# NeuralRevenant/RASSEngine

Measured on AMD Instinct MI355X. Metric: queries/sec, exact cosine top-10 over N x 1024-d fp32 corpus in HBM, higher is better.
Workload: dtype f32; 1 GPU; 1000000 x 1024-d flat cosine top-10, 1 x MI355X, precomputed embeddings (BASELINE configs[1]); rows_per_gpu=1000000, rows_global=1000000, dim=1024, k=10, query_batch=32, corpus_dtype=f32, layout=tile16, mode=flat

## Files before the change

rassengine_amd/csrc/api_internal.h:

```cpp
#pragma once

#include <hip/hip_runtime.h>
#include <stdint.h>
#include <stdio.h>
#include <stdlib.h>
#include <string.h>
#include <unistd.h>

#include <algorithm>
#include <atomic>
#include <condition_variable>
#include <map>
#include <mutex>
#include <new>
#include <string>
#include <type_traits>
#include <vector>

#include "../../include/rass_engine.h"
#include "kernels.h"

namespace rass {
namespace host {

// ... 334 lines not shown
    int64_t* d_pair_ids = nullptr;
    unsigned char* d_batch = nullptr;
    size_t batch_bytes = 0;
    unsigned char* d_allow_ws = nullptr;
    size_t allow_ws_bytes = 0;
};

namespace rass {
namespace host {

int set_device(const rass_engine* eng);
int index_reserve(rass_index* idx, int64_t need_rows);
void index_free_slabs(rass_index* idx);
int index_attr_ensure(rass_index* idx, int col);
int index_refresh_copies(rass_index* idx, int64_t first, int64_t n, hipStream_t st);

int scan_xcd_skew(int nq, int grid, int n_cus);
int64_t scan_sample_floor_min_share();
bool i8_sample_floor(int64_t rows, int grid);
enum { kBatchSampleGroups = 0, kBatchSampleF32 = 1, kBatchSampleRep = 2 };
int scan_batch_sample_mode();
bool scan_batch_pair();
bool scan_batch_step();
bool ivf_batch_one_launch();

int scan_grid(int64_t tiles, int lists_kept_per_wg, int n_cus);

template <class F>
int timed_launch(rass_engine* eng, hipStream_t st, F&& launch, int extra_groups = 0) {
    const bool timed = eng && eng->ev_on && (size_t)(2 * eng->ev_used + 1) < eng->ev_pool.size();
    if (timed) HIP_TRY(hipEventRecord(eng->ev_pool[2 * eng->ev_used], st));
    const int rc = launch();
    if (rc != RASS_OK) return rc;
    if (timed) {
        HIP_TRY(hipEventRecord(eng->ev_pool[2 * eng->ev_used + 1], st));
        eng->ev_used += 1;
        eng->ev_extra += extra_groups;
    }
    return RASS_OK;
}

inline void as_sample(rass::ScanArgs& s) { s.xcd_skew = 0, s.sample_pass = true; }
inline void as_sample(rass::ScanBf16Args& s) { s.k = 1; }
inline void as_sample(rass::ScanI8Args& s) { s.k = 1; }
template <class Args>
int sample_prelaunch(Args& a, int grid, float* best, hipError_t (*launch)(const Args&, int, hipStream_t), hipStream_t st,
// ... 174 lines not shown
```

rassengine_amd/csrc/api_scan.hip:

```cpp

#include "api_internal.h"

namespace rass {
namespace host {


int scan_xcd_skew(int nq, int grid, int n_cus) {
    struct Skew {
        int b16 = 4, b32 = 0;
        Skew() {
            if (const char* e = getenv("RASS_SCAN_XCD_SKEW")) {
                int a = 0, b = 0;
                const int n = sscanf(e, "%d,%d", &a, &b);
                if (n == 1) b = a;
                if (n >= 1 && a >= 0 && b >= 0 && a <= 4096 && b <= 4096) b16 = a, b32 = b;
            }
        }
    };
    if (grid != n_cus || grid % 8 != 0) return 0;
    static const Skew skew;
    return nq <= 16 ? skew.b16 : skew.b32;
}

int64_t scan_sample_floor_min_share() {
// ... 9 lines not shown
    if (e && !force && atoi(e) == 0) return false;
    return grid <= rass::kMaxSampleGroups && rows >= (int64_t)(force ? 2 : 8) * 64 * grid;
}

int scan_batch_sample_mode() {
    const char* e = getenv("RASS_SCAN_BATCH_SAMPLE");
    if (e && e[0] == 'g') return kBatchSampleGroups;
    if (e && e[0] == 'f') return kBatchSampleF32;
    return kBatchSampleRep;
}

bool scan_batch_pair() {
    static const bool on = [] {
        const char* e = getenv("RASS_SCAN_BATCH_PAIR");
        return !(e && e[0] == '0');
    }();
    return on;
}

bool scan_batch_step() {
    const char* e = getenv("RASS_SCAN_BATCH_STEP");
    return !(e && e[0] == '0');
}

bool ivf_batch_one_launch() {
    const char* e = getenv("RASS_IVF_BATCH_FINE");
    return !(e && e[0] == 'g');
}


int scan_grid(int64_t tiles, int lists_kept_per_wg, int n_cus) {
    int grid = (int)std::min<int64_t>(std::max<int64_t>(tiles, 1), std::min(n_cus, kMaxGrid));
    if ((int64_t)grid * lists_kept_per_wg > rass::kMergeMaxCandidates) grid = rass::kMergeMaxCandidates / lists_kept_per_wg;
    return grid;
}

ScratchView scratch_layout(unsigned char* base, int nq, int k) {
    Carver c{base};
    ScratchView L;
    L.q_padded = c.take<float>((size_t)RASS_MAX_QBATCH * kMaxStride * sizeof(float));
    L.part_scores = c.take<float>((size_t)kMaxGrid * nq * k * sizeof(float));
    L.part_ids = c.take<int64_t>((size_t)kMaxGrid * nq * k * sizeof(int64_t));
    L.q_bf16 = c.take<unsigned short>((size_t)RASS_MAX_QBATCH * kMaxStride * 2);
    L.cand_scores = c.take<float>((size_t)RASS_MAX_QBATCH * RASS_MAX_K * sizeof(float));
    L.cand_ids = c.take<int64_t>((size_t)RASS_MAX_QBATCH * RASS_MAX_K * sizeof(int64_t));
    L.sample_best = c.take<float>((size_t)rass::kMaxSampleGroups * 32 * sizeof(float));
// ... 436 lines not shown
```

rassengine_amd/csrc/api_search.hip:

```cpp

#include "api_internal.h"

namespace rass {
namespace host {

HostSlot* slot_acquire(rass_engine* eng) {
    std::unique_lock<std::mutex> lk(eng->slot_mu);
    for (;;) {
        for (HostSlot& sl : eng->slots)
            if (!sl.busy) {
                sl.busy = true;
                return &sl;
            }
        eng->slot_cv.wait(lk);
    }
}

void slot_release(rass_engine* eng, HostSlot* sl) {
    {
        std::lock_guard<std::mutex> lk(eng->slot_mu);
        sl->busy = false;
    }
    eng->slot_cv.notify_one();
}
// ... 81 lines not shown
    hipStream_t st = eng->stream;
    const int nq = r.nq, k = r.k;
    const IndexView iv = index_view(idx, r.q_filter != nullptr, r.id_base);
    const int64_t rows = iv.rows;
    const int64_t stride = idx->stride;
    if (int rc = check_k(k)) return rc;
    if (rows < 0 || rows > kMaxScanRows) return fail(RASS_ERR_INVALID, "n_rows out of range for one scan");
    if (!rass::scan_supported_stride(stride) || stride > kMaxStride)
        return fail(RASS_ERR_UNSUPPORTED, kStrideMsg);
    const int groups = (nq + RASS_MAX_QBATCH - 1) / RASS_MAX_QBATCH;
    if (stride > kNarrowStride) {
        for (int g = 0; g < groups; ++g) {
            const int rc = search_device_group(idx, batch_group(idx, r, g, gs, gi));
            if (rc != RASS_OK) return rc;
        }
        return RASS_OK;
    }
    const BatchSamplePlan plan = batch_sample_plan(eng, rows, stride, nq, k);
    const int grid = plan.grid;
    int rc = grow_block(&eng->d_batch, &eng->batch_bytes, batch_layout(nullptr, groups, grid, k, stride).total, st);
    if (rc != RASS_OK) return rc;
    const BatchView L = batch_layout(eng->d_batch, groups, grid, k, stride);

    HIP_TRY(rass::launch_normalize_rows_f32(r.queries, idx->dim, L.q_padded, stride, nq, idx->dim, st, (int64_t)groups * 32));

    auto group_args = [&](int g) {
        rass::ScanArgs a;
        a.corpus = iv.corpus;
        a.row_tag = iv.row_tag;
        a.q_padded = L.q_padded + (int64_t)g * 32 * stride;
        a.q_filter = r.q_filter ? r.q_filter + g * 32 : nullptr;
        a.part_scores = L.part_scores + (int64_t)g * L.part_per_group;
        a.part_ids = L.part_ids + (int64_t)g * L.part_per_group;
        a.row_stride = stride;
        a.id_base = iv.id_base;
        a.n_rows = (int)rows;
        a.nq = std::min(RASS_MAX_QBATCH, nq - g * 32);
        a.k = k;
        a.xcd_skew = scan_xcd_skew(a.nq, grid, eng->n_cus);
        return a;
    };
    const int64_t sample_rows = (int64_t)64 * grid;
    const bool sample = plan.sample, one_sample = plan.one_sample;
    const int sample_wgs = one_sample ? 32 : grid;
    if (plan.rep) {
        HIP_TRY(rass::launch_sample_rep(iv.corpus, iv.row_tag, stride, grid, L.q_padded, r.q_filter, nq, L.rep_qfrag, L.rep_part,
                                        L.rep_row, L.sample_best, st));
    } else if (one_sample) {
        rass::ScanArgs s = group_args(0);
        s.n_rows = (int)sample_rows;
        s.xcd_skew = 0;
        s.sample_pass = true;
        s.nq = 32;
        s.part_scores = L.sample_best;
        s.part_ids = nullptr;
        s.wgs_per_group = sample_wgs;
        s.q_group_stride = 32 * stride;
        s.part_group_stride = (int64_t)32 * rass::kMaxSampleGroups;
        s.nq_total = nq;
        HIP_TRY(rass::launch_scan_topk_f32(s, groups * sample_wgs, st));
    } else if (sample)
        for (int g = 0; g < groups; ++g) {
            rass::ScanArgs a = group_args(g);
            if (a.nq <= 16) continue;
            rc = sample_prelaunch(a, grid, L.group_sample(g), rass::launch_scan_topk_f32, st);
            if (rc != RASS_OK) return rc;
        }
    const bool pairs = scan_batch_pair() && rass::scan_pair_supported_stride(stride);
    const int n_pairs = pairs ? nq / (2 * RASS_MAX_QBATCH) : 0;
    const bool step = scan_batch_step() && n_pairs >= 2 && grid <= (rows + 31) / 32;
// ... 25 lines not shown
            rc = timed_launch(eng, st, [&] { return HIP_RC(rass::launch_scan_topk_f32(a, grid, st)); });
        if (rc != RASS_OK) return rc;
    }
    const rass::MergeGroups mg = dense_groups(nq, (int64_t)L.part_per_group, gs, gi);
    HIP_TRY(rass::launch_merge_topk(L.part_scores, L.part_ids, grid, nq, k, r.out_scores, r.out_ids, st, iv.id_map, 0, 0, &mg));
    return RASS_OK;
}

int sample_floor_hook(rass_index* idx, const float* d_queries, int nq, int k, const int32_t* d_q_filter, int32_t* d_rows,
                      float* d_scores, float* d_floors = nullptr) {
    rass_engine* eng = idx->eng;
    hipStream_t st = eng->stream;
    const IndexView iv = index_view(idx, d_q_filter != nullptr, 0);
    const int64_t stride = idx->stride;
    if (idx->dtype != RASS_F32 || idx->prefilter || nq <= RASS_MAX_QBATCH || iv.rows <= 0 || iv.rows > kMaxScanRows ||
        stride > kNarrowStride || !rass::scan_supported_stride(stride))
        return fail(RASS_ERR_UNSUPPORTED, "not a fused fp32 batch");
    const BatchSamplePlan plan = batch_sample_plan(eng, iv.rows, stride, nq, k);
    if (!plan.rep) return fail(RASS_ERR_UNSUPPORTED, "this batch does not take the representatives' sample stage");
    const int groups = nq / RASS_MAX_QBATCH;
    int rc = grow_block(&eng->d_batch, &eng->batch_bytes, batch_layout(nullptr, groups, plan.grid, k, stride).total, st);
    if (rc != RASS_OK) return rc;
    const BatchView L = batch_layout(eng->d_batch, groups, plan.grid, k, stride);
    HIP_TRY(rass::launch_normalize_rows_f32(d_queries, idx->dim, L.q_padded, stride, nq, idx->dim, st, nq));
    HIP_TRY(rass::launch_sample_rep(iv.corpus, iv.row_tag, stride, plan.grid, L.q_padded, d_q_filter, nq, L.rep_qfrag, L.rep_part,
                                    L.rep_row, L.sample_best, st));
    if (d_floors) {
        HIP_TRY(rass::launch_step_floors(L.sample_best, 32, nq, k, L.step_floor, st));
        HIP_TRY(hipMemcpyAsync(d_floors, L.step_floor, (size_t)nq * sizeof(float), hipMemcpyDeviceToDevice, st));
        return RASS_OK;
    }
    HIP_TRY(hipMemcpyAsync(d_rows, L.rep_row, (size_t)nq * 32 * sizeof(int32_t), hipMemcpyDeviceToDevice, st));
    HIP_TRY(hipMemcpy2DAsync(d_scores, 32 * sizeof(float), L.sample_best, rass::kMaxSampleGroups * sizeof(float), 32 * sizeof(float),
                             (size_t)nq, hipMemcpyDeviceToDevice, st));
    return RASS_OK;
}

int prefilter_launch_batch(rass_index* idx, const FlatRequest& r, int64_t gs, int64_t gi) {
    rass_engine* eng = idx->eng;
    hipStream_t st = eng->stream;
    const int nq = r.nq;
    const IndexView iv = index_view(idx, r.q_filter != nullptr, r.id_base);
    const int64_t rows = iv.rows;
    const int64_t stride = idx->stride;
    const int kc = RASS_MAX_K;
    const int groups = (nq + RASS_MAX_QBATCH - 1) / RASS_MAX_QBATCH;
    const int grid = scan_grid((rows + 63) / 64, kc, eng->n_cus);
    int rc = grow_block(&eng->d_batch, &eng->batch_bytes, batch_layout(nullptr, groups, grid, kc, stride, true).total, st);
    if (rc != RASS_OK) return rc;
// ... 403 lines not shown
```

rassengine_amd/csrc/exact_score.h:

```cpp
#pragma once

#include <hip/hip_runtime.h>
#include <stdint.h>

#include "scan_core.h"

namespace rass {

template <int CH, int HALVES>
__device__ __forceinline__ float flat_score_slice(const float* __restrict__ slab, int64_t stride, const float* __restrict__ q_padded,
                                                  int q, int64_t row, int w) {
    float acc = 0.f;
#pragma unroll
    for (int half = 0; half < HALVES; ++half) {
        const float* xb = slab + (row >> 4) * 16 * stride + (int64_t)(w * HALVES * CH + half * CH) * 256 + (int)(row & 15) * 4;
        const float* qv = q_padded + (int64_t)q * stride + (w * HALVES * CH + half * CH) * 16;
        f32x4 xv[CH][4];
#pragma unroll
        for (int j = 0; j < CH; ++j)
#pragma unroll
            for (int g = 0; g < 4; ++g) xv[j][g] = *reinterpret_cast<const f32x4*>(xb + j * 256 + g * 64);
#pragma unroll
        for (int j = 0; j < CH; ++j) {
            f32x4 qq[4];
#pragma unroll
            for (int g = 0; g < 4; ++g) qq[g] = *reinterpret_cast<const f32x4*>(qv + j * 16 + 4 * g);
#pragma unroll
            for (int i = 0; i < 4; ++i)
#pragma unroll
                for (int g = 0; g < 4; ++g) acc = fmaf(xv[j][g][i], qq[g][i], acc);
        }
    }
    return acc;
}

}
```

rassengine_amd/csrc/kernels.h:

```cpp
#pragma once

#include <hip/hip_runtime.h>
#include <stddef.h>
#include <stdint.h>

namespace rass {

constexpr int kMaxSampleGroups = 256;

struct ScanArgs {
    const float* corpus;
    const int32_t* row_tag;
    const float* q_padded;
    const int32_t* q_filter;
    const int32_t* q_filter_mask = nullptr;
    const float* q_after_score = nullptr;
    const int64_t* q_after_id = nullptr;
    float* part_scores;
    int64_t* part_ids;
    int64_t row_stride;
    int64_t id_base;
    int n_rows;
    int nq;
    int k;
// ... 204 lines not shown
    int nq;
    int k;
    int64_t id_base = 0;
    const int32_t* q_filter_mask = nullptr;
    const float* q_after_score = nullptr;
    const int64_t* q_after_id = nullptr;
    const int32_t* work_tile = nullptr;
    const int32_t* work_rows = nullptr;
    const uint32_t* work_mask = nullptr;
    const int32_t* n_work = nullptr;
    const float* sample_best = nullptr;
    int sample_groups = 0;
};
hipError_t launch_scan_bf16_topk(const ScanBf16Args& a, int grid, hipStream_t stream);
hipError_t launch_convert_tile16_bf16(const float* src, void* dst, int64_t stride, int64_t block0, int64_t block1,
                                      hipStream_t stream, int64_t src_block0 = -1, int64_t row_lo = 0,
                                      int64_t row_hi = -1);
hipError_t launch_unpack_rows_tile16b(const void* slab, int64_t stride, int64_t first_row, int64_t n, int dim,
                                      float* out, int64_t out_stride, hipStream_t stream);
hipError_t launch_queries_to_bf16(const float* src, void* dst, int64_t n, hipStream_t stream);
bool sample_rep_supported(int64_t stride, int grid);
hipError_t launch_sample_rep(const float* slab, const int32_t* row_tag, int64_t stride, int grid, const float* q_padded,
                             const int32_t* q_filter, int nq, void* q_frag, void* rep_part, int* rep_row, float* sample_best,
                             hipStream_t stream);
hipError_t launch_step_floors(const float* sample_best, int sample_groups, int nq, int k, float* floors, hipStream_t stream);
hipError_t launch_rerank_f32(const float* slab, int64_t stride, const float* q_padded, const int64_t* cand_rows, int nq,
                             int n_cand, int k, int64_t id_base, float* out_scores, int64_t* out_ids,
                             hipStream_t stream, int64_t out_scores_group_stride = 0, int64_t out_ids_group_stride = 0,
                             const int64_t* id_map = nullptr);

struct ScanI8Args {
    const signed char* corpus;
    const float* row_scale;
    const int32_t* row_tag;
    const signed char* q_i8;
    const int32_t* q_filter;
    float* part_scores;
    int64_t* part_ids;
    int64_t row_stride;
    int n_rows;
    int nq;
    int k;
    const float* sample_best = nullptr;
    int sample_groups = 0;
    const int32_t* q_filter_mask = nullptr;
    int wgs_per_group = 0;
    int64_t q_group_stride = 0, part_group_stride = 0;
// ... 160 lines not shown
```

rassengine_amd/csrc/merge_topk.hip:

```cpp

#include <hip/hip_runtime.h>
#include <stdint.h>

#include "kernels.h"
#include "scan_core.h"

namespace rass {

constexpr int kMergeWaves = 16;
constexpr int kMergeThreads = kMergeWaves * 64;
constexpr int64_t kWorstId = 0x7fffffffffffffffLL;

struct Cand {
    float s;
    int64_t id;
};

__device__ __forceinline__ bool cand_better(const Cand& a, const Cand& b) {
    return (a.s > b.s) || (a.s == b.s && a.id < b.id);
}

template <int STRIDE>
__device__ __forceinline__ Cand xor_cand(const Cand& c, int lane) {
    Cand o;
    o.s = __int_as_float(xor_lane<STRIDE>(__float_as_int(c.s), lane));
    const int lo = xor_lane<STRIDE>((int)(c.id & 0xffffffffLL), lane);
    const int hi = xor_lane<STRIDE>((int)(c.id >> 32), lane);
    o.id = ((int64_t)hi << 32) | (uint32_t)lo;
    return o;
}

__device__ __forceinline__ Cand reverse_cand(const Cand& c, int lane) {
    Cand o = xor_cand<32>(c, lane);
    o = xor_cand<16>(o, lane);
    o.s = __int_as_float(__builtin_amdgcn_mov_dpp(__float_as_int(o.s), 0x140, 0xf, 0xf, true));
    const int lo = __builtin_amdgcn_mov_dpp((int)(o.id & 0xffffffffLL), 0x140, 0xf, 0xf, true);
    const int hi = __builtin_amdgcn_mov_dpp((int)(o.id >> 32), 0x140, 0xf, 0xf, true);
    o.id = ((int64_t)hi << 32) | (uint32_t)lo;
    return o;
}

template <int STRIDE>
__device__ __forceinline__ void cmpx(Cand& c, int lane, bool keep_better) {
    const Cand o = xor_cand<STRIDE>(c, lane);
    const bool mine_better = cand_better(c, o);
    if (mine_better != keep_better) c = o;
}

template <int SIZE, int STRIDE>
__device__ __forceinline__ void sort_steps(Cand& c, int lane) {
    if constexpr (STRIDE > 0) {
        const bool best_first = (lane & SIZE) == 0;
        const bool lower = (lane & STRIDE) == 0;
        cmpx<STRIDE>(c, lane, best_first == lower);
        sort_steps<SIZE, STRIDE / 2>(c, lane);
    }
}

__device__ __forceinline__ void wave_sort64(Cand& c, int lane) {
    sort_steps<2, 1>(c, lane);
    sort_steps<4, 2>(c, lane);
    sort_steps<8, 4>(c, lane);
    sort_steps<16, 8>(c, lane);
    sort_steps<32, 16>(c, lane);
    sort_steps<64, 32>(c, lane);
}

template <int STRIDE>
__device__ __forceinline__ void merge_steps(Cand& c, int lane) {
    if constexpr (STRIDE > 0) {
        cmpx<STRIDE>(c, lane, (lane & STRIDE) == 0);
        merge_steps<STRIDE / 2>(c, lane);
    }
}
__device__ __forceinline__ void wave_bitonic_merge64(Cand& c, int lane) { merge_steps<32>(c, lane); }

__device__ __forceinline__ void fold_group(Cand& run, const Cand& grp_sorted, int lane) {
    const Cand rev = reverse_cand(grp_sorted, lane);
    Cand c = (lane < 32) ? run : rev;
    wave_bitonic_merge64(c, lane);
    run = c;
}

__global__ __launch_bounds__(kMergeThreads) void merge_topk_kernel(const float* __restrict__ scores,
                                                                   const int64_t* __restrict__ ids, int n_lists,
                                                                   int , int k, float* __restrict__ out_scores,
                                                                   int64_t* __restrict__ out_ids,
                                                                   const int64_t* __restrict__ id_map,
                                                                   int64_t score_list_stride, int64_t id_list_stride,
                                                                   MergeGroups grp, const int32_t* __restrict__ live_nq) {
    if (live_nq != nullptr && __builtin_amdgcn_readfirstlane(*live_nq) == 0) return;
    __shared__ float sh_s[kMergeWaves * 32];
    __shared__ int64_t sh_i[kMergeWaves * 32];
    int q = blockIdx.x;
    if (grp.size > 0) {
        const int g = q / grp.size;
        q -= g * grp.size;
        scores += (int64_t)g * grp.score_stride;
        ids += (int64_t)g * grp.id_stride;
        out_scores += (int64_t)g * grp.out_score_stride;
        out_ids += (int64_t)g * grp.out_id_stride;
        if (grp.lists_are_dense) {
            const int nq_g = min(grp.size, grp.nq_total - g * grp.size);
            score_list_stride = id_list_stride = (int64_t)nq_g * k;
        }
    }
    const int lane = threadIdx.x & 63;
    const int wave = threadIdx.x >> 6;
    const int n = n_lists * k;

    Cand run;
    run.s = -INFINITY;
    run.id = kWorstId;
    for (int base = wave * 64; base < n; base += kMergeWaves * 64) {
        const int e = base + lane;
        Cand c;
        c.s = -INFINITY;
        c.id = kWorstId;
        if (e < n) {
            const int list = e / k, kk = e - list * k;
            const int64_t o = (int64_t)q * k + kk;
            const int64_t gi = ids[(int64_t)list * id_list_stride + o];
            const float gs = scores[(int64_t)list * score_list_stride + o];
            if (gi >= 0 && gs > -INFINITY) {
                c.s = gs;
                c.id = gi;
            }
        }
        wave_sort64(c, lane);
        fold_group(run, c, lane);
    }
    Cand acc = run;
#pragma unroll 1
    for (int step = 1; step < kMergeWaves; step <<= 1) {
        const bool sender = (wave & (2 * step - 1)) == step;
        const bool receiver = (wave & (2 * step - 1)) == 0;
        if (sender && lane < 32) {
            sh_s[wave * 32 + lane] = acc.s;
            sh_i[wave * 32 + lane] = acc.id;
        }
        __syncthreads();
        if (receiver) {
            Cand c;
            c.s = sh_s[(wave + step) * 32 + (31 - (lane & 31))];
            c.id = sh_i[(wave + step) * 32 + (31 - (lane & 31))];
            if (lane < 32) c = acc;
            wave_bitonic_merge64(c, lane);
            acc = c;
        }
    }
    if (wave != 0) return;
    if (lane < k) {
        const bool filled = acc.id != kWorstId;
        out_scores[(int64_t)q * k + lane] = filled ? acc.s : -INFINITY;
        out_ids[(int64_t)q * k + lane] = filled ? (id_map ? id_map[acc.id] : acc.id) : (int64_t)-1;
    }
}

hipError_t launch_merge_topk(const float* scores, const int64_t* ids, int n_lists, int nq, int k,
                             float* out_scores, int64_t* out_ids, hipStream_t stream, const int64_t* id_map,
                             int64_t score_list_stride, int64_t id_list_stride, const MergeGroups* groups,
                             const int32_t* live_nq) {
    const int64_t n = (int64_t)n_lists * k;
    if (n_lists < 1 || nq < 1 || k < 1 || k > 32 || n > kMergeMaxCandidates) return hipErrorInvalidValue;
    if (score_list_stride <= 0) score_list_stride = (int64_t)nq * k;
    if (id_list_stride <= 0) id_list_stride = (int64_t)nq * k;
    MergeGroups grp;
    if (groups) {
        grp = *groups;
        if (grp.size < 1 || grp.nq_total != nq) return hipErrorInvalidValue;
    }
    hipLaunchKernelGGL(merge_topk_kernel, dim3(nq), dim3(kMergeThreads), 0, stream, scores, ids, n_lists, nq, k,
                       out_scores, out_ids, id_map, score_list_stride, id_list_stride, grp, live_nq);
    return hipGetLastError();
}

constexpr int kRangeFinishThreads = 1024;

__device__ __forceinline__ unsigned range_score_key(unsigned bits) {
    if (bits == 0x80000000u) bits = 0u;
    return (bits & 0x80000000u) ? ~bits : (bits | 0x80000000u);
}

__global__ __launch_bounds__(kRangeFinishThreads) void range_finish_kernel(const unsigned* __restrict__ count,
                                                                             const uint2* __restrict__ hits, int cap, int64_t id_base,
                                                                             const int64_t* __restrict__ id_map,
                                                                             float* __restrict__ out_scores, int64_t* __restrict__ out_ids,
                                                                             int64_t* __restrict__ total) {
    __shared__ unsigned long long keys[kRangeMaxHits];
    const int q = blockIdx.x, tid = threadIdx.x;
    const unsigned cnt = count[q * kRangeCountStride];
    if (tid == 0) total[q] = (int64_t)cnt;
    float* os = out_scores + (int64_t)q * cap;
    int64_t* oi = out_ids + (int64_t)q * cap;
    const int n = cnt > (unsigned)cap ? 0 : (int)cnt;
    int n2 = 1;
// ... 48 lines not shown
```

rassengine_amd/csrc/rowops.hip:

```cpp

#include <hip/hip_runtime.h>
#include <stdint.h>

#include "kernels.h"

namespace rass {

typedef float f32x4 __attribute__((ext_vector_type(4)));

constexpr int kRowThreads = 256;

__device__ __forceinline__ float wave_sum(float v) {
#pragma unroll
    for (int off = 32; off > 0; off >>= 1) v += __shfl_xor(v, off, 64);
    return v;
}

__global__ __launch_bounds__(kRowThreads) void normalize_rows_kernel(const float* __restrict__ in,
                                                                     int64_t in_stride, float* __restrict__ out,
                                                                     int64_t out_stride, int64_t n, int dim,
                                                                     int64_t n_total) {
    const int lane = threadIdx.x & 63;
    const int wave = threadIdx.x >> 6;
    for (int64_t r = n + (int64_t)blockIdx.x * 4 + wave; r < n_total; r += (int64_t)gridDim.x * 4) {
        float* dst = out + r * out_stride;
        for (int c = lane; c < (int)out_stride; c += 64) dst[c] = 0.f;
    }
    const bool vec = ((dim & 3) == 0) && ((in_stride & 3) == 0) && ((out_stride & 3) == 0) &&
                     ((reinterpret_cast<uintptr_t>(in) & 15) == 0) && ((reinterpret_cast<uintptr_t>(out) & 15) == 0);
    for (int64_t r = (int64_t)blockIdx.x * 4 + wave; r < n; r += (int64_t)gridDim.x * 4) {
        const float* src = in + r * in_stride;
        float* dst = out + r * out_stride;
        float ss = 0.f;
        if (vec) {
            for (int c = lane * 4; c < dim; c += 256) {
                const f32x4 v = *reinterpret_cast<const f32x4*>(src + c);
                ss = fmaf(v.x, v.x, ss);
                ss = fmaf(v.y, v.y, ss);
                ss = fmaf(v.z, v.z, ss);
                ss = fmaf(v.w, v.w, ss);
            }
        } else {
            for (int c = lane; c < dim; c += 64) ss = fmaf(src[c], src[c], ss);
        }
        ss = wave_sum(ss);
        const float denom = sqrtf(ss) + 1e-9f;
        if (vec) {
            for (int c = lane * 4; c < (int)out_stride; c += 256) {
                f32x4 v = f32x4{0.f, 0.f, 0.f, 0.f};
                if (c < dim) {
                    v = *reinterpret_cast<const f32x4*>(src + c);
                    v.x = v.x / denom;
                    v.y = v.y / denom;
                    v.z = v.z / denom;
                    v.w = v.w / denom;
                }
                *reinterpret_cast<f32x4*>(dst + c) = v;
            }
        } else {
            for (int c = lane; c < (int)out_stride; c += 64) dst[c] = (c < dim) ? src[c] / denom : 0.f;
        }
    }
}

hipError_t launch_normalize_rows_f32(const float* in, int64_t in_stride, float* out, int64_t out_stride,
                                     int64_t n, int dim, hipStream_t stream, int64_t n_total) {
    if (n_total < n) n_total = n;
    if (n_total <= 0) return hipSuccess;
    int64_t blocks = (n_total + 3) / 4;
    if (blocks > 256 * 16) blocks = 256 * 16;
    hipLaunchKernelGGL(normalize_rows_kernel, dim3((unsigned)blocks), dim3(kRowThreads), 0, stream, in, in_stride,
                       out, out_stride, n, dim, n_total);
    return hipGetLastError();
}

__global__ void zero_rows_kernel(float* dst, int64_t total) {
    for (int64_t i = (int64_t)blockIdx.x * blockDim.x + threadIdx.x; i < total; i += (int64_t)gridDim.x * blockDim.x)
        dst[i] = 0.f;
}

hipError_t launch_zero_rows(float* dst, int64_t stride, int n_rows, hipStream_t stream) {
    const int64_t total = stride * n_rows;
    if (total <= 0) return hipSuccess;
    int64_t blocks = (total + 255) / 256;
    if (blocks > 1024) blocks = 1024;
// ... 269 lines not shown
```

rassengine_amd/csrc/sample_rep.hip:

```cpp

#include <hip/hip_runtime.h>
#include <limits.h>
#include <stdint.h>

#include "kernels.h"
#include "scan_core.h"
#include "exact_score.h"

namespace rass {

typedef __bf16 bf16x8 __attribute__((ext_vector_type(8)));
typedef __bf16 bf16x4 __attribute__((ext_vector_type(4)));

constexpr int kRepThreads = 512;
constexpr int kRepRows = 64;

__device__ __forceinline__ bf16x8 pack_bf16(const f32x4 a, const f32x4 b) {
    const bf16x4 lo = __builtin_convertvector(a, bf16x4), hi = __builtin_convertvector(b, bf16x4);
    return __builtin_shufflevector(lo, hi, 0, 1, 2, 3, 4, 5, 6, 7);
}

__device__ __forceinline__ void take_better(float& s, int& r, float os, int orow) {
    const bool take = (os > s) | ((os == s) & (orow < r));
    s = take ? os : s;
    r = take ? orow : r;
}

__global__ __launch_bounds__(256) void sample_queries_frag_kernel(const float* __restrict__ q_padded, int64_t stride,
                                                                  bf16x8* __restrict__ q_frag, int n_frag) {
    const int i = blockIdx.x * 256 + threadIdx.x;
    if (i >= n_frag) return;
    const int ks_per_tile = (int)(stride >> 5);
    const int lane = i & 63, ks = (i >> 6) % ks_per_tile, tile = (i >> 6) / ks_per_tile;
    const float* src = q_padded + (int64_t)(tile * 16 + (lane & 15)) * stride + 32 * ks + 4 * (lane >> 4);
    q_frag[i] = pack_bf16(*reinterpret_cast<const f32x4*>(src), *reinterpret_cast<const f32x4*>(src + 16));
}

template <int CH>
__global__ __launch_bounds__(kRepThreads, 2) void sample_rep_bf16_kernel(const float* __restrict__ slab,
                                                                         const int32_t* __restrict__ row_tag,
                                                                         const bf16x8* __restrict__ q_frag,
                                                                         const int32_t* __restrict__ q_filter, int n_tiles,
                                                                         int2* __restrict__ rep_part) {
    constexpr int KS = 4 * CH;
    constexpr int64_t stride = 128 * CH;
    __shared__ bf16x8 rows[KS * 4 * 64];
    const int lane = threadIdx.x & 63;
    const int wid = __builtin_amdgcn_readfirstlane(threadIdx.x >> 6);
    const int g = lane >> 4;
    const int row0 = blockIdx.x * kRepRows;

    {
        const float* base = slab + (int64_t)row0 * stride + lane * 4;
#pragma unroll
        for (int half = 0; half < 2; ++half) {
            f32x4 v[CH][2];
#pragma unroll
            for (int u = 0; u < CH; ++u) {
// ... 58 lines not shown
            __builtin_amdgcn_sched_barrier(0);
        }
        const int qfil = q_filter ? qraw : -1;
        float bs = -INFINITY;
        int br = INT_MAX;
#pragma unroll
        for (int rb = 0; rb < 4; ++rb)
#pragma unroll
            for (int r = 0; r < 4; ++r) {
                const int tg = tag[rb][r];
                const bool ok = (tg != -1) & ((qfil < 0) | (qfil == tg));
                const float s = acc[rb][r];
                const bool take = ok & (s > bs);
                bs = take ? s : bs;
                br = take ? row0 + 16 * rb + 4 * g + r : br;
            }
        take_better(bs, br, __int_as_float(xor_lane<16>(__float_as_int(bs), lane)), xor_lane<16>(br, lane));
        take_better(bs, br, __int_as_float(xor_lane<32>(__float_as_int(bs), lane)), xor_lane<32>(br, lane));
        if (lane < 16) rep_part[(int64_t)q * gridDim.x + blockIdx.x] = make_int2(__float_as_int(bs), br);
        t += 8;
    } while (t < n_tiles);
}

template <int CH>
__global__ __launch_bounds__(256) __attribute__((amdgpu_waves_per_eu(1, 2))) void sample_rescore_f32_kernel(const float* __restrict__ slab,
                                                                 const float* __restrict__ q_padded,
                                                                 const int2* __restrict__ rep_part, int grid, int n_groups,
                                                                 int* __restrict__ rep_row, float* __restrict__ sample_best) {
    constexpr int64_t stride = 128 * CH;
    __shared__ float part[32][9];
    __shared__ int rw[32];
    const int x = blockIdx.x & 7, j = blockIdx.x >> 3;
    const int c = threadIdx.x >> 3, w = threadIdx.x & 7;
    const int subs = grid >> 5;
    const int lane = lane_id();
    if (j >= n_groups) return;
    auto pick = [&](int b, int grp) {
        float bs = -INFINITY;
        int br = INT_MAX;
        if (w < subs) {
            const int2 v = rep_part[(int64_t)(grp * 32 + c) * grid + b * subs + w];
            bs = __int_as_float(v.x), br = v.y;
        }
        take_better(bs, br, __int_as_float(xor_lane<1>(__float_as_int(bs), lane)), xor_lane<1>(br, lane));
        take_better(bs, br, __int_as_float(xor_lane<2>(__float_as_int(bs), lane)), xor_lane<2>(br, lane));
        take_better(bs, br, __int_as_float(xor_lane<4>(__float_as_int(bs), lane)), xor_lane<4>(br, lane));
        return br == INT_MAX ? -1 : br;
    };
    int b = x, grp = j;
    int row = pick(b, grp);
    for (;;) {
        int nb = b, ng = grp + 32;
        if (ng >= n_groups) nb = b + 8, ng = j;
        const bool more = nb < 32;
        const int row_next = more ? pick(nb, ng) : -1;
        float acc = 0.f;
        if (row >= 0) acc = flat_score_slice<CH, 1>(slab, stride, q_padded, grp * 32 + c, row, w);
        part[c][w] = acc;
        if (w == 0) rw[c] = row;
        __syncthreads();
        if (threadIdx.x < 32) {
            const int cc = threadIdx.x, qq = grp * 32 + cc;
            float s = part[cc][0];
#pragma unroll
            for (int ww = 1; ww < 8; ++ww) s += part[cc][ww];
            const int r = rw[cc];
            const bool ok = r >= 0 && fabsf(s) < INFINITY;
            sample_best[(int64_t)qq * kMaxSampleGroups + b] = ok ? s : -INFINITY;
            rep_row[qq * 32 + b] = r;
        }
        if (!more) break;
        __syncthreads();
        b = nb, grp = ng, row = row_next;
    }
}

bool sample_rep_supported(int64_t stride, int grid) {
    return stride >= 128 && stride <= 1024 && stride % 128 == 0 && grid >= 32 && grid % 32 == 0 && grid <= kMaxSampleGroups;
}

hipError_t launch_sample_rep(const float* slab, const int32_t* row_tag, int64_t stride, int grid, const float* q_padded,
                             const int32_t* q_filter, int nq, void* q_frag, void* rep_part, int* rep_row, float* sample_best,
                             hipStream_t stream) {
    if (!sample_rep_supported(stride, grid) || nq < 32 || nq % 32 != 0) return hipErrorInvalidValue;
    bf16x8* const qf = static_cast<bf16x8*>(q_frag);
    int2* const part = static_cast<int2*>(rep_part);
    const int n_frag = (int)((int64_t)nq * stride / 8);
    hipLaunchKernelGGL(sample_queries_frag_kernel, dim3((n_frag + 255) / 256), dim3(256), 0, stream, q_padded, stride, qf, n_frag);
#define RASS_REP_CASE(C)                                                                                                      \
    case C:                                                                                                                   \
        hipLaunchKernelGGL(sample_rep_bf16_kernel<C>, dim3(grid), dim3(kRepThreads), 0, stream, slab, row_tag, qf, q_filter,  \
                           nq / 16, part);                                                                                    \
        hipLaunchKernelGGL(sample_rescore_f32_kernel<C>, dim3(256), dim3(256), 0, stream, slab, q_padded, part, grid, nq / 32, \
                           rep_row, sample_best);                                                                             \
        break;
    switch ((int)(stride >> 7)) {
        RASS_REP_CASE(1) RASS_REP_CASE(2) RASS_REP_CASE(3) RASS_REP_CASE(4)
        RASS_REP_CASE(5) RASS_REP_CASE(6) RASS_REP_CASE(7) RASS_REP_CASE(8)
        default: return hipErrorInvalidValue;
    }
#undef RASS_REP_CASE
    return hipGetLastError();
}

__global__ __launch_bounds__(256) void step_floors_kernel(const float* __restrict__ sample_best, int sample_groups, int nq, int k,
                                                          float* __restrict__ floors) {
    const int lane = lane_id();
    const int q = blockIdx.x * 4 + (threadIdx.x >> 6);
    if (q >= nq) return;
    unsigned key[kMaxSampleGroups / 64];
#pragma unroll
    for (int j = 0; j < kMaxSampleGroups / 64; ++j) {
        const int grp = lane + 64 * j;
        const float v = grp < sample_groups ? sample_best[(int64_t)q * kMaxSampleGroups + grp] : -INFINITY;
        key[j] = v == -INFINITY ? 0u : score_key(v);
    }
    unsigned T = 0;
// ... 19 lines not shown
```

Measured before the change: 58380 queries/s.

## Fuse query prep with bf16 frag packing, stage rescore queries in LDS, add select merge

```diff
diff --git a/rassengine_amd/csrc/api_internal.h b/rassengine_amd/csrc/api_internal.h
--- a/rassengine_amd/csrc/api_internal.h
+++ b/rassengine_amd/csrc/api_internal.h
@@ -380,6 +380,7 @@
 int scan_batch_sample_mode();
 bool scan_batch_pair();
 bool scan_batch_step();
+bool scan_batch_prep_fused();
 bool ivf_batch_one_launch();
 
 int scan_grid(int64_t tiles, int lists_kept_per_wg, int n_cus);
diff --git a/rassengine_amd/csrc/api_scan.hip b/rassengine_amd/csrc/api_scan.hip
--- a/rassengine_amd/csrc/api_scan.hip
+++ b/rassengine_amd/csrc/api_scan.hip
@@ -55,6 +55,12 @@
     const char* e = getenv("RASS_SCAN_BATCH_STEP");
     return !(e && e[0] == '0');
 }
+
+bool scan_batch_prep_fused() {
+    const char* e = getenv("RASS_SCAN_BATCH_PREP");
+    return !(e && e[0] == 's');
+}
+
 
 bool ivf_batch_one_launch() {
     const char* e = getenv("RASS_IVF_BATCH_FINE");
diff --git a/rassengine_amd/csrc/api_search.hip b/rassengine_amd/csrc/api_search.hip
--- a/rassengine_amd/csrc/api_search.hip
+++ b/rassengine_amd/csrc/api_search.hip
@@ -127,7 +127,9 @@
     if (rc != RASS_OK) return rc;
     const BatchView L = batch_layout(eng->d_batch, groups, grid, k, stride);
 
-    HIP_TRY(rass::launch_normalize_rows_f32(r.queries, idx->dim, L.q_padded, stride, nq, idx->dim, st, (int64_t)groups * 32));
+    const bool fused_prep = plan.rep && scan_batch_prep_fused();
+    if (fused_prep) HIP_TRY(rass::launch_sample_prep(r.queries, idx->dim, idx->dim, L.q_padded, stride, nq, L.rep_qfrag, st));
+    else HIP_TRY(rass::launch_normalize_rows_f32(r.queries, idx->dim, L.q_padded, stride, nq, idx->dim, st, (int64_t)groups * 32));
 
     auto group_args = [&](int g) {
         rass::ScanArgs a;
@@ -150,7 +152,7 @@
     const int sample_wgs = one_sample ? 32 : grid;
     if (plan.rep) {
         HIP_TRY(rass::launch_sample_rep(iv.corpus, iv.row_tag, stride, grid, L.q_padded, r.q_filter, nq, L.rep_qfrag, L.rep_part,
-                                        L.rep_row, L.sample_best, st));
+                                        L.rep_row, L.sample_best, st, fused_prep));
     } else if (one_sample) {
         rass::ScanArgs s = group_args(0);
         s.n_rows = (int)sample_rows;
@@ -222,9 +224,11 @@
     int rc = grow_block(&eng->d_batch, &eng->batch_bytes, batch_layout(nullptr, groups, plan.grid, k, stride).total, st);
     if (rc != RASS_OK) return rc;
     const BatchView L = batch_layout(eng->d_batch, groups, plan.grid, k, stride);
-    HIP_TRY(rass::launch_normalize_rows_f32(d_queries, idx->dim, L.q_padded, stride, nq, idx->dim, st, nq));
+    const bool fused_prep = scan_batch_prep_fused();
+    if (fused_prep) HIP_TRY(rass::launch_sample_prep(d_queries, idx->dim, idx->dim, L.q_padded, stride, nq, L.rep_qfrag, st));
+    else HIP_TRY(rass::launch_normalize_rows_f32(d_queries, idx->dim, L.q_padded, stride, nq, idx->dim, st, nq));
     HIP_TRY(rass::launch_sample_rep(iv.corpus, iv.row_tag, stride, plan.grid, L.q_padded, d_q_filter, nq, L.rep_qfrag, L.rep_part,
-                                    L.rep_row, L.sample_best, st));
+                                    L.rep_row, L.sample_best, st, fused_prep));
     if (d_floors) {
         HIP_TRY(rass::launch_step_floors(L.sample_best, 32, nq, k, L.step_floor, st));
         HIP_TRY(hipMemcpyAsync(d_floors, L.step_floor, (size_t)nq * sizeof(float), hipMemcpyDeviceToDevice, st));
diff --git a/rassengine_amd/csrc/exact_score.h b/rassengine_amd/csrc/exact_score.h
--- a/rassengine_amd/csrc/exact_score.h
+++ b/rassengine_amd/csrc/exact_score.h
@@ -34,4 +34,27 @@
     return acc;
 }
 
+template <int CH>
+__device__ __forceinline__ float flat_score_slice_at(const float* __restrict__ slab, int64_t stride, const float* __restrict__ qslice,
+                                                     int64_t row, int w) {
+    float acc = 0.f;
+    const float* xb = slab + (row >> 4) * 16 * stride + (int64_t)(w * CH) * 256 + (int)(row & 15) * 4;
+    f32x4 xv[CH][4];
+#pragma unroll
+    for (int j = 0; j < CH; ++j)
+#pragma unroll
+        for (int g = 0; g < 4; ++g) xv[j][g] = *reinterpret_cast<const f32x4*>(xb + j * 256 + g * 64);
+#pragma unroll
+    for (int j = 0; j < CH; ++j) {
+        f32x4 qq[4];
+#pragma unroll
+        for (int g = 0; g < 4; ++g) qq[g] = *reinterpret_cast<const f32x4*>(qslice + j * 16 + 4 * g);
+#pragma unroll
+        for (int i = 0; i < 4; ++i)
+#pragma unroll
+            for (int g = 0; g < 4; ++g) acc = fmaf(xv[j][g][i], qq[g][i], acc);
+    }
+    return acc;
 }
+
+}
diff --git a/rassengine_amd/csrc/kernels.h b/rassengine_amd/csrc/kernels.h
--- a/rassengine_amd/csrc/kernels.h
+++ b/rassengine_amd/csrc/kernels.h
@@ -250,7 +250,9 @@
 bool sample_rep_supported(int64_t stride, int grid);
 hipError_t launch_sample_rep(const float* slab, const int32_t* row_tag, int64_t stride, int grid, const float* q_padded,
                              const int32_t* q_filter, int nq, void* q_frag, void* rep_part, int* rep_row, float* sample_best,
-                             hipStream_t stream);
+                             hipStream_t stream, bool frag_ready = false);
+hipError_t launch_sample_prep(const float* queries, int64_t in_stride, int dim, float* q_padded, int64_t stride, int nq, void* q_frag,
+                              hipStream_t stream);
 hipError_t launch_step_floors(const float* sample_best, int sample_groups, int nq, int k, float* floors, hipStream_t stream);
 hipError_t launch_rerank_f32(const float* slab, int64_t stride, const float* q_padded, const int64_t* cand_rows, int nq,
                              int n_cand, int k, int64_t id_base, float* out_scores, int64_t* out_ids,
diff --git a/rassengine_amd/csrc/merge_topk.hip b/rassengine_amd/csrc/merge_topk.hip
--- a/rassengine_amd/csrc/merge_topk.hip
+++ b/rassengine_amd/csrc/merge_topk.hip
@@ -1,6 +1,7 @@
 
 #include <hip/hip_runtime.h>
 #include <stdint.h>
+#include <stdlib.h>
 
 #include "kernels.h"
 #include "scan_core.h"
@@ -8,7 +9,8 @@
 namespace rass {
 
 constexpr int kMergeWaves = 16;
-constexpr int kMergeThreads = kMergeWaves * 64;
+constexpr int kSelectWaves = 4;
+constexpr int kSelectCap = 256;
 constexpr int64_t kWorstId = 0x7fffffffffffffffLL;
 
 struct Cand {
@@ -40,15 +42,25 @@
     return o;
 }
 
+__device__ __forceinline__ bool cand_better(float a, float b) { return a > b; }
 template <int STRIDE>
-__device__ __forceinline__ void cmpx(Cand& c, int lane, bool keep_better) {
-    const Cand o = xor_cand<STRIDE>(c, lane);
+__device__ __forceinline__ float xor_cand(float v, int lane) {
+    return __int_as_float(xor_lane<STRIDE>(__float_as_int(v), lane));
+}
+__device__ __forceinline__ float reverse_cand(float v, int lane) {
+    const float o = xor_cand<16>(xor_cand<32>(v, lane), lane);
+    return __int_as_float(__builtin_amdgcn_mov_dpp(__float_as_int(o), 0x140, 0xf, 0xf, true));
+}
+
+template <int STRIDE, class T>
+__device__ __forceinline__ void cmpx(T& c, int lane, bool keep_better) {
+    const T o = xor_cand<STRIDE>(c, lane);
     const bool mine_better = cand_better(c, o);
     if (mine_better != keep_better) c = o;
 }
 
-template <int SIZE, int STRIDE>
-__device__ __forceinline__ void sort_steps(Cand& c, int lane) {
+template <int SIZE, int STRIDE, class T>
+__device__ __forceinline__ void sort_steps(T& c, int lane) {
     if constexpr (STRIDE > 0) {
         const bool best_first = (lane & SIZE) == 0;
         const bool lower = (lane & STRIDE) == 0;
@@ -57,7 +69,8 @@
     }
 }
 
-__device__ __forceinline__ void wave_sort64(Cand& c, int lane) {
+template <class T>
+__device__ __forceinline__ void wave_sort64(T& c, int lane) {
     sort_steps<2, 1>(c, lane);
     sort_steps<4, 2>(c, lane);
     sort_steps<8, 4>(c, lane);
@@ -66,32 +79,35 @@
     sort_steps<64, 32>(c, lane);
 }
 
-template <int STRIDE>
-__device__ __forceinline__ void merge_steps(Cand& c, int lane) {
+template <int STRIDE, class T>
+__device__ __forceinline__ void merge_steps(T& c, int lane) {
     if constexpr (STRIDE > 0) {
         cmpx<STRIDE>(c, lane, (lane & STRIDE) == 0);
         merge_steps<STRIDE / 2>(c, lane);
     }
 }
-__device__ __forceinline__ void wave_bitonic_merge64(Cand& c, int lane) { merge_steps<32>(c, lane); }
-
-__device__ __forceinline__ void fold_group(Cand& run, const Cand& grp_sorted, int lane) {
-    const Cand rev = reverse_cand(grp_sorted, lane);
-    Cand c = (lane < 32) ? run : rev;
+template <class T>
+__device__ __forceinline__ void wave_bitonic_merge64(T& c, int lane) { merge_steps<32>(c, lane); }
+
+template <class T>
+__device__ __forceinline__ void fold_group(T& run, const T& grp_sorted, int lane) {
+    const T rev = reverse_cand(grp_sorted, lane);
+    T c = (lane < 32) ? run : rev;
     wave_bitonic_merge64(c, lane);
     run = c;
 }
 
-__global__ __launch_bounds__(kMergeThreads) void merge_topk_kernel(const float* __restrict__ scores,
-                                                                   const int64_t* __restrict__ ids, int n_lists,
-                                                                   int , int k, float* __restrict__ out_scores,
-                                                                   int64_t* __restrict__ out_ids,
-                                                                   const int64_t* __restrict__ id_map,
-                                                                   int64_t score_list_stride, int64_t id_list_stride,
-                                                                   MergeGroups grp, const int32_t* __restrict__ live_nq) {
+template <int WAVES, bool SELECT>
+__global__ __launch_bounds__(WAVES * 64) void merge_topk_kernel(const float* __restrict__ scores,
+                                                                const int64_t* __restrict__ ids, int n_lists,
+                                                                int , int k, float* __restrict__ out_scores,
+                                                                int64_t* __restrict__ out_ids,
+                                                                const int64_t* __restrict__ id_map,
+                                                                int64_t score_list_stride, int64_t id_list_stride,
+                                                                MergeGroups grp, const int32_t* __restrict__ live_nq) {
     if (live_nq != nullptr && __builtin_amdgcn_readfirstlane(*live_nq) == 0) return;
-    __shared__ float sh_s[kMergeWaves * 32];
-    __shared__ int64_t sh_i[kMergeWaves * 32];
+    __shared__ float sh_s[WAVES * 32];
+    __shared__ int64_t sh_i[WAVES * 32];
     int q = blockIdx.x;
     if (grp.size > 0) {
         const int g = q / grp.size;
@@ -109,44 +125,124 @@
     const int wave = threadIdx.x >> 6;
     const int n = n_lists * k;
 
-    Cand run;
-    run.s = -INFINITY;
-    run.id = kWorstId;
-    for (int base = wave * 64; base < n; base += kMergeWaves * 64) {
-        const int e = base + lane;
-        Cand c;
-        c.s = -INFINITY;
-        c.id = kWorstId;
-        if (e < n) {
+    Cand acc;
+    acc.s = -INFINITY;
+    acc.id = kWorstId;
+    bool sort_all = true;
+    if constexpr (SELECT) {
+        extern __shared__ float sh_all[];
+        __shared__ float sh_t[WAVES * 32];
+        __shared__ float sh_cs[kSelectCap];
+        __shared__ int64_t sh_ci[kSelectCap];
+        __shared__ int sh_cnt;
+        if (threadIdx.x == 0) sh_cnt = 0;
+#pragma unroll 4
+        for (int e = threadIdx.x; e < n; e += WAVES * 64) {
             const int list = e / k, kk = e - list * k;
             const int64_t o = (int64_t)q * k + kk;
             const int64_t gi = ids[(int64_t)list * id_list_stride + o];
             const float gs = scores[(int64_t)list * score_list_stride + o];
-            if (gi >= 0 && gs > -INFINITY) {
-                c.s = gs;
-                c.id = gi;
-            }
-        }
-        wave_sort64(c, lane);
-        fold_group(run, c, lane);
-    }
-    Cand acc = run;
+            sh_all[e] = (gi >= 0 && gs > -INFINITY) ? gs : -INFINITY;
+        }
+        __syncthreads();
+        float run = -INFINITY;
+        for (int base = wave * 64; base < n_lists; base += WAVES * 64) {
+            const int list = base + lane;
+            float m = -INFINITY;
+            if (list < n_lists)
+                for (int kk = 0; kk < k; ++kk) m = fmaxf(m, sh_all[list * k + kk]);
+            wave_sort64(m, lane);
+            fold_group(run, m, lane);
+        }
+        if (lane < 32) sh_t[wave * 32 + lane] = run;
+        __syncthreads();
+        float top = -INFINITY;
+        for (int w = 0; w < WAVES && w * 64 < n_lists; ++w) {
+            const float other = sh_t[w * 32 + (31 - (lane & 31))];
+            float c = (lane < 32) ? top : other;
+            wave_bitonic_merge64(c, lane);
+            top = c;
+        }
+        const float t = __shfl(top, k - 1, 64);
+        for (int e = threadIdx.x; e < n; e += WAVES * 64) {
+            const float s = sh_all[e];
+            if (s >= t && s > -INFINITY) {
+                const int pos = atomicAdd(&sh_cnt, 1);
+                if (pos < kSelectCap) {
+                    const int list = e / k, kk = e - list * k;
+                    sh_cs[pos] = s;
+                    sh_ci[pos] = ids[(int64_t)list * id_list_stride + (int64_t)q * k + kk];
+                }
+            }
+        }
+        __syncthreads();
+        const int cnt = sh_cnt;
+        sort_all = cnt > kSelectCap;
+        if (!sort_all) {
+            const int e = wave * 64 + lane;
+            if (e < cnt) {
+                acc.s = sh_cs[e];
+                acc.id = sh_ci[e];
+            }
+            if (wave * 64 < cnt) wave_sort64(acc, lane);
+            if (cnt > 64) {
+                if (wave > 0 && lane < 32) {
+                    sh_s[wave * 32 + lane] = acc.s;
+                    sh_i[wave * 32 + lane] = acc.id;
+                }
+                __syncthreads();
+                if (wave == 0)
+                    for (int w = 1; w * 64 < cnt; ++w) {
+                        Cand c;
+                        c.s = sh_s[w * 32 + (31 - (lane & 31))];
+                        c.id = sh_i[w * 32 + (31 - (lane & 31))];
+                        if (lane < 32) c = acc;
+                        wave_bitonic_merge64(c, lane);
+                        acc = c;
+                    }
+            }
+        }
+    }
+    if (sort_all) {
+        Cand run;
+        run.s = -INFINITY;
+        run.id = kWorstId;
+        for (int base = wave * 64; base < n; base += WAVES * 64) {
+            const int e = base + lane;
+            Cand c;
+            c.s = -INFINITY;
+            c.id = kWorstId;
+            if (e < n) {
+                const int list = e / k, kk = e - list * k;
+                const int64_t o = (int64_t)q * k + kk;
+                const int64_t gi = ids[(int64_t)list * id_list_stride + o];
+                const float gs = scores[(int64_t)list * score_list_stride + o];
+                if (gi >= 0 && gs > -INFINITY) {
+                    c.s = gs;
+                    c.id = gi;
+                }
+            }
+            wave_sort64(c, lane);
+            fold_group(run, c, lane);
+        }
+        acc = run;
 #pragma unroll 1
-    for (int step = 1; step < kMergeWaves; step <<= 1) {
-        const bool sender = (wave & (2 * step - 1)) == step;
-        const bool receiver = (wave & (2 * step - 1)) == 0;
-        if (sender && lane < 32) {
-            sh_s[wave * 32 + lane] = acc.s;
-            sh_i[wave * 32 + lane] = acc.id;
-        }
-        __syncthreads();
-        if (receiver) {
-            Cand c;
-            c.s = sh_s[(wave + step) * 32 + (31 - (lane & 31))];
-            c.id = sh_i[(wave + step) * 32 + (31 - (lane & 31))];
-            if (lane < 32) c = acc;
-            wave_bitonic_merge64(c, lane);
-            acc = c;
+        for (int step = 1; step < WAVES; step <<= 1) {
+            const bool sender = (wave & (2 * step - 1)) == step;
+            const bool receiver = (wave & (2 * step - 1)) == 0;
+            if (sender && lane < 32) {
+                sh_s[wave * 32 + lane] = acc.s;
+                sh_i[wave * 32 + lane] = acc.id;
+            }
+            __syncthreads();
+            if (receiver) {
+                Cand c;
+                c.s = sh_s[(wave + step) * 32 + (31 - (lane & 31))];
+                c.id = sh_i[(wave + step) * 32 + (31 - (lane & 31))];
+                if (lane < 32) c = acc;
+                wave_bitonic_merge64(c, lane);
+                acc = c;
+            }
         }
     }
     if (wave != 0) return;
@@ -155,6 +251,11 @@
         out_scores[(int64_t)q * k + lane] = filled ? acc.s : -INFINITY;
         out_ids[(int64_t)q * k + lane] = filled ? (id_map ? id_map[acc.id] : acc.id) : (int64_t)-1;
     }
+}
+
+static bool merge_select() {
+    const char* e = getenv("RASS_MERGE_SELECT");
+    return !(e && e[0] == '0');
 }
 
 hipError_t launch_merge_topk(const float* scores, const int64_t* ids, int n_lists, int nq, int k,
@@ -170,8 +271,15 @@
         grp = *groups;
         if (grp.size < 1 || grp.nq_total != nq) return hipErrorInvalidValue;
     }
-    hipLaunchKernelGGL(merge_topk_kernel, dim3(nq), dim3(kMergeThreads), 0, stream, scores, ids, n_lists, nq, k,
-                       out_scores, out_ids, id_map, score_list_stride, id_list_stride, grp, live_nq);
+    if (merge_select()) {
+        const auto kern = merge_topk_kernel<kSelectWaves, true>;
+        hipLaunchKernelGGL(kern, dim3(nq), dim3(kSelectWaves * 64), (size_t)n * sizeof(float), stream, scores, ids, n_lists, nq, k,
+                           out_scores, out_ids, id_map, score_list_stride, id_list_stride, grp, live_nq);
+    } else {
+        const auto kern = merge_topk_kernel<kMergeWaves, false>;
+        hipLaunchKernelGGL(kern, dim3(nq), dim3(kMergeWaves * 64), 0, stream, scores, ids, n_lists, nq, k,
+                           out_scores, out_ids, id_map, score_list_stride, id_list_stride, grp, live_nq);
+    }
     return hipGetLastError();
 }
 
diff --git a/rassengine_amd/csrc/rowops.h b/rassengine_amd/csrc/rowops.h
--- /dev/null
+++ b/rassengine_amd/csrc/rowops.h
@@ -0,0 +1,65 @@
+#pragma once
+
+#include <hip/hip_runtime.h>
+#include <stdint.h>
+
+namespace rass {
+
+typedef float f32x4 __attribute__((ext_vector_type(4)));
+
+__device__ __forceinline__ float wave_sum(float v) {
+#pragma unroll
+    for (int off = 32; off > 0; off >>= 1) v += __shfl_xor(v, off, 64);
+    return v;
+}
+
+struct NoRowSink {
+    __device__ __forceinline__ void operator()(int, const f32x4&) const {}
+    __device__ __forceinline__ void operator()(int, float) const {}
+};
+
+template <class Sink>
+__device__ __forceinline__ void normalize_row(const float* __restrict__ src, float* __restrict__ dst, int dim, int out_stride,
+                                              int lane, bool vec, const Sink& sink) {
+    float ss = 0.f;
+    if (vec) {
+        for (int c = lane * 4; c < dim; c += 256) {
+            const f32x4 v = *reinterpret_cast<const f32x4*>(src + c);
+            ss = fmaf(v.x, v.x, ss);
+            ss = fmaf(v.y, v.y, ss);
+            ss = fmaf(v.z, v.z, ss);
+            ss = fmaf(v.w, v.w, ss);
+        }
+    } else {
+        for (int c = lane; c < dim; c += 64) ss = fmaf(src[c], src[c], ss);
+    }
+    ss = wave_sum(ss);
+    const float denom = sqrtf(ss) + 1e-9f;
+    if (vec) {
+        for (int c = lane * 4; c < out_stride; c += 256) {
+            f32x4 v = f32x4{0.f, 0.f, 0.f, 0.f};
+            if (c < dim) {
+                v = *reinterpret_cast<const f32x4*>(src + c);
+                v.x = v.x / denom;
+                v.y = v.y / denom;
+                v.z = v.z / denom;
+                v.w = v.w / denom;
+            }
+            *reinterpret_cast<f32x4*>(dst + c) = v;
+            sink(c, v);
+        }
+    } else {
+        for (int c = lane; c < out_stride; c += 64) {
+            const float v = (c < dim) ? src[c] / denom : 0.f;
+            dst[c] = v;
+            sink(c, v);
+        }
+    }
+}
+
+__device__ __forceinline__ bool rows_vec_ok(const float* in, int64_t in_stride, const float* out, int64_t out_stride, int dim) {
+    return ((dim & 3) == 0) && ((in_stride & 3) == 0) && ((out_stride & 3) == 0) &&
+           ((reinterpret_cast<uintptr_t>(in) & 15) == 0) && ((reinterpret_cast<uintptr_t>(out) & 15) == 0);
+}
+
+}
diff --git a/rassengine_amd/csrc/rowops.hip b/rassengine_amd/csrc/rowops.hip
--- a/rassengine_amd/csrc/rowops.hip
+++ b/rassengine_amd/csrc/rowops.hip
@@ -3,18 +3,11 @@
 #include <stdint.h>
 
 #include "kernels.h"
+#include "rowops.h"
 
 namespace rass {
 
-typedef float f32x4 __attribute__((ext_vector_type(4)));
-
 constexpr int kRowThreads = 256;
-
-__device__ __forceinline__ float wave_sum(float v) {
-#pragma unroll
-    for (int off = 32; off > 0; off >>= 1) v += __shfl_xor(v, off, 64);
-    return v;
-}
 
 __global__ __launch_bounds__(kRowThreads) void normalize_rows_kernel(const float* __restrict__ in,
                                                                      int64_t in_stride, float* __restrict__ out,
@@ -26,41 +19,9 @@
         float* dst = out + r * out_stride;
         for (int c = lane; c < (int)out_stride; c += 64) dst[c] = 0.f;
     }
-    const bool vec = ((dim & 3) == 0) && ((in_stride & 3) == 0) && ((out_stride & 3) == 0) &&
-                     ((reinterpret_cast<uintptr_t>(in) & 15) == 0) && ((reinterpret_cast<uintptr_t>(out) & 15) == 0);
-    for (int64_t r = (int64_t)blockIdx.x * 4 + wave; r < n; r += (int64_t)gridDim.x * 4) {
-        const float* src = in + r * in_stride;
-        float* dst = out + r * out_stride;
-        float ss = 0.f;
-        if (vec) {
-            for (int c = lane * 4; c < dim; c += 256) {
-                const f32x4 v = *reinterpret_cast<const f32x4*>(src + c);
-                ss = fmaf(v.x, v.x, ss);
-                ss = fmaf(v.y, v.y, ss);
-                ss = fmaf(v.z, v.z, ss);
-                ss = fmaf(v.w, v.w, ss);
-            }
-        } else {
-            for (int c = lane; c < dim; c += 64) ss = fmaf(src[c], src[c], ss);
-        }
-        ss = wave_sum(ss);
-        const float denom = sqrtf(ss) + 1e-9f;
-        if (vec) {
-            for (int c = lane * 4; c < (int)out_stride; c += 256) {
-                f32x4 v = f32x4{0.f, 0.f, 0.f, 0.f};
-                if (c < dim) {
-                    v = *reinterpret_cast<const f32x4*>(src + c);
-                    v.x = v.x / denom;
-                    v.y = v.y / denom;
-                    v.z = v.z / denom;
-                    v.w = v.w / denom;
-                }
-                *reinterpret_cast<f32x4*>(dst + c) = v;
-            }
-        } else {
-            for (int c = lane; c < (int)out_stride; c += 64) dst[c] = (c < dim) ? src[c] / denom : 0.f;
-        }
-    }
+    const bool vec = rows_vec_ok(in, in_stride, out, out_stride, dim);
+    for (int64_t r = (int64_t)blockIdx.x * 4 + wave; r < n; r += (int64_t)gridDim.x * 4)
+        normalize_row(in + r * in_stride, out + r * out_stride, dim, (int)out_stride, lane, vec, NoRowSink{});
 }
 
 hipError_t launch_normalize_rows_f32(const float* in, int64_t in_stride, float* out, int64_t out_stride,
diff --git a/rassengine_amd/csrc/sample_rep.hip b/rassengine_amd/csrc/sample_rep.hip
--- a/rassengine_amd/csrc/sample_rep.hip
+++ b/rassengine_amd/csrc/sample_rep.hip
@@ -6,6 +6,7 @@
 #include "kernels.h"
 #include "scan_core.h"
 #include "exact_score.h"
+#include "rowops.h"
 
 namespace rass {
 
@@ -34,6 +35,38 @@
     const int lane = i & 63, ks = (i >> 6) % ks_per_tile, tile = (i >> 6) / ks_per_tile;
     const float* src = q_padded + (int64_t)(tile * 16 + (lane & 15)) * stride + 32 * ks + 4 * (lane >> 4);
     q_frag[i] = pack_bf16(*reinterpret_cast<const f32x4*>(src), *reinterpret_cast<const f32x4*>(src + 16));
+}
+
+struct FragSink {
+    bf16x8* q_frag;
+    int row, ks_per_tile;
+    __device__ __forceinline__ __bf16* slot(int c) const {
+        const int64_t i = ((int64_t)(row >> 4) * ks_per_tile + (c >> 5)) * 64 + (row & 15) + 16 * ((c >> 2) & 3);
+        return reinterpret_cast<__bf16*>(q_frag + i) + 4 * ((c >> 4) & 1) + (c & 3);
+    }
+    __device__ __forceinline__ void operator()(int c, const f32x4& v) const {
+        *reinterpret_cast<bf16x4*>(slot(c)) = __builtin_convertvector(v, bf16x4);
+    }
+    __device__ __forceinline__ void operator()(int c, float v) const { *slot(c) = (__bf16)v; }
+};
+
+__global__ __launch_bounds__(256) void sample_prep_kernel(const float* __restrict__ in, int64_t in_stride, float* __restrict__ q_padded,
+                                                          int64_t stride, int nq, int dim, bf16x8* __restrict__ q_frag) {
+    const int lane = threadIdx.x & 63;
+    const int wave = threadIdx.x >> 6;
+    const bool vec = rows_vec_ok(in, in_stride, q_padded, stride, dim);
+    for (int r = blockIdx.x * 4 + wave; r < nq; r += gridDim.x * 4)
+        normalize_row(in + (int64_t)r * in_stride, q_padded + (int64_t)r * stride, dim, (int)stride, lane, vec,
+                      FragSink{q_frag, r, (int)(stride >> 5)});
+}
+
+hipError_t launch_sample_prep(const float* queries, int64_t in_stride, int dim, float* q_padded, int64_t stride, int nq, void* q_frag,
+                              hipStream_t stream) {
+    if (stride < 128 || stride % 128 != 0 || dim < 1 || dim > stride || in_stride < dim || nq < 16 || nq % 16 != 0)
+        return hipErrorInvalidValue;
+    hipLaunchKernelGGL(sample_prep_kernel, dim3((nq + 3) / 4), dim3(256), 0, stream, queries, in_stride, q_padded, stride, nq, dim,
+                       static_cast<bf16x8*>(q_frag));
+    return hipGetLastError();
 }
 
 template <int CH>
@@ -138,12 +171,17 @@
     } while (t < n_tiles);
 }
 
+constexpr int rescore_slice_floats(int ch) { return 16 * ch + 4; }
+constexpr int rescore_query_floats(int ch) { return 8 * rescore_slice_floats(ch) + 4; }
+constexpr size_t rescore_lds_bytes(int ch) { return (size_t)32 * rescore_query_floats(ch) * sizeof(float); }
 template <int CH>
 __global__ __launch_bounds__(256) __attribute__((amdgpu_waves_per_eu(1, 2))) void sample_rescore_f32_kernel(const float* __restrict__ slab,
                                                                  const float* __restrict__ q_padded,
                                                                  const int2* __restrict__ rep_part, int grid, int n_groups,
                                                                  int* __restrict__ rep_row, float* __restrict__ sample_best) {
     constexpr int64_t stride = 128 * CH;
+    constexpr int SS = rescore_slice_floats(CH), QS = rescore_query_floats(CH);
+    extern __shared__ float qs[];
     __shared__ float part[32][9];
     __shared__ int rw[32];
     const int x = blockIdx.x & 7, j = blockIdx.x >> 3;
@@ -163,15 +201,25 @@
         take_better(bs, br, __int_as_float(xor_lane<4>(__float_as_int(bs), lane)), xor_lane<4>(br, lane));
         return br == INT_MAX ? -1 : br;
     };
-    int b = x, grp = j;
+    int b = x, grp = j, staged = -1;
     int row = pick(b, grp);
     for (;;) {
         int nb = b, ng = grp + 32;
         if (ng >= n_groups) nb = b + 8, ng = j;
         const bool more = nb < 32;
         const int row_next = more ? pick(nb, ng) : -1;
+        if (grp != staged) {
+            const f32x4* src = reinterpret_cast<const f32x4*>(q_padded + (int64_t)grp * 32 * stride);
+#pragma unroll 8
+            for (int i = threadIdx.x; i < 32 * 32 * CH; i += 256) {
+                const int qc = i / (32 * CH), col4 = i % (32 * CH);
+                *reinterpret_cast<f32x4*>(qs + qc * QS + (col4 / (4 * CH)) * SS + (col4 % (4 * CH)) * 4) = src[i];
+            }
+            __syncthreads();
+            staged = grp;
+        }
         float acc = 0.f;
-        if (row >= 0) acc = flat_score_slice<CH, 1>(slab, stride, q_padded, grp * 32 + c, row, w);
+        if (row >= 0) acc = flat_score_slice_at<CH>(slab, stride, qs + c * QS + w * SS, row, w);
         part[c][w] = acc;
         if (w == 0) rw[c] = row;
         __syncthreads();
@@ -191,24 +239,38 @@
     }
 }
 
+template <int CH>
+static hipError_t rescore_allow_lds() {
+    static bool attr_set = false;
+    if (!attr_set) {
+        hipError_t e = hipFuncSetAttribute(reinterpret_cast<const void*>(&sample_rescore_f32_kernel<CH>),
+                                           hipFuncAttributeMaxDynamicSharedMemorySize, (int)rescore_lds_bytes(CH));
+        if (e != hipSuccess) return e;
+        attr_set = true;
+    }
+    return hipSuccess;
+}
+
 bool sample_rep_supported(int64_t stride, int grid) {
     return stride >= 128 && stride <= 1024 && stride % 128 == 0 && grid >= 32 && grid % 32 == 0 && grid <= kMaxSampleGroups;
 }
 
 hipError_t launch_sample_rep(const float* slab, const int32_t* row_tag, int64_t stride, int grid, const float* q_padded,
                              const int32_t* q_filter, int nq, void* q_frag, void* rep_part, int* rep_row, float* sample_best,
-                             hipStream_t stream) {
+                             hipStream_t stream, bool frag_ready) {
     if (!sample_rep_supported(stride, grid) || nq < 32 || nq % 32 != 0) return hipErrorInvalidValue;
     bf16x8* const qf = static_cast<bf16x8*>(q_frag);
     int2* const part = static_cast<int2*>(rep_part);
     const int n_frag = (int)((int64_t)nq * stride / 8);
-    hipLaunchKernelGGL(sample_queries_frag_kernel, dim3((n_frag + 255) / 256), dim3(256), 0, stream, q_padded, stride, qf, n_frag);
+    if (!frag_ready)
+        hipLaunchKernelGGL(sample_queries_frag_kernel, dim3((n_frag + 255) / 256), dim3(256), 0, stream, q_padded, stride, qf, n_frag);
 #define RASS_REP_CASE(C)                                                                                                      \
     case C:                                                                                                                   \
         hipLaunchKernelGGL(sample_rep_bf16_kernel<C>, dim3(grid), dim3(kRepThreads), 0, stream, slab, row_tag, qf, q_filter,  \
                            nq / 16, part);                                                                                    \
-        hipLaunchKernelGGL(sample_rescore_f32_kernel<C>, dim3(256), dim3(256), 0, stream, slab, q_padded, part, grid, nq / 32, \
-                           rep_row, sample_best);                                                                             \
+        if (hipError_t e = rescore_allow_lds<C>(); e != hipSuccess) return e;                                                 \
+        hipLaunchKernelGGL(sample_rescore_f32_kernel<C>, dim3(256), dim3(256), rescore_lds_bytes(C), stream, slab, q_padded,  \
+                           part, grid, nq / 32, rep_row, sample_best);                                                        \
         break;
     switch ((int)(stride >> 7)) {
         RASS_REP_CASE(1) RASS_REP_CASE(2) RASS_REP_CASE(3) RASS_REP_CASE(4)
```

Result: no change. 58550 queries/s (median of 6 runs) (+0.3%).
